# tdj28/ml-depth-pro-video

Measured on AMD Instinct MI355X. Metric: frames/sec at 1536x1536 (1/2/4/8 MI355X) + depth L1 vs reference, higher is better.
Workload: dtype bf16+f16; 1 GPU; BASELINE config 2/3: one 1536x1536 frame per GPU per step through DepthPro.infer (patch+image+FOV ViT-L, decoder, heads), hipGraph replay; global_batch=1, parallelism=frame-dp1, graph=True

## Files before the change

### ml-depth-pro-video_amd/csrc/dp_gemm.hip

```cpp
#include "dp_gemm_impl.h"

namespace dpg {
std::atomic<int> g_dbg_flags{0};

constexpr int DP_MAX_DEV = 64;
std::atomic<int> g_num_cu[DP_MAX_DEV];
int num_cus() {
  int dev = 0;
  if (hipGetDevice(&dev) != hipSuccess || dev < 0) dev = 0;
  std::atomic<int>& slot = g_num_cu[dev < DP_MAX_DEV ? dev : 0];
  int n = slot.load(std::memory_order_relaxed);
  if (n <= 0) {
    if (hipDeviceGetAttribute(&n, hipDeviceAttributeMultiprocessorCount, dev) != hipSuccess || n <= 0) n = 256;
    if (dev < DP_MAX_DEV) slot.store(n, std::memory_order_relaxed);
  }
  return n;
}
}

namespace {
int launch_tile(const GemmP& p, int tile, bool conv, bool bf16, hipStream_t s) {
  switch (tile) {
    case DP_TILE_PBIG_320x256: case DP_TILE_PBIG_256x256: return launch_part_pbig(p, tile, conv, bf16, s);
    case DP_TILE_256x64: case DP_TILE_256x32: case DP_TILE_128x128: case DP_TILE_DUAL_256x128:
// ... 19 lines not shown

namespace {
__global__ void ws_check_kernel(uint32_t* __restrict__ ws, int32_t* __restrict__ status) {
  const uint32_t err = ws[DP_GEMM_WS_ERROR_OFFSET / 4];
  if (threadIdx.x == 0) status[0] = (int32_t)err;
  if (err == 0) return;
  __syncthreads();
  for (int i = threadIdx.x; i < (int)(SK_FLAG_BYTES / 4); i += blockDim.x) ws[i] = 0u;
}
}

extern "C" int dp_gemm_workspace_check(void* workspace, int32_t* status, dp_stream_t stream) {
  if (!workspace || !status) return DP_ERR_ARG;
  hipLaunchKernelGGL(ws_check_kernel, dim3(1), dim3(256), 0, (hipStream_t)stream, (uint32_t*)workspace, status);
  DP_CHECK_LAUNCH();
  return 0;
}

namespace {
int gemm_plan(const dp_gemm_args* a, GemmP& p, int& tile) {
  if (!a) return DP_ERR_ARG;
  if (a->M <= 0 || a->N <= 0 || a->K <= 0) return DP_ERR_SHAPE;
  if (a->K % BK != 0 || a->N % 4 != 0) return DP_ERR_SHAPE;
  if (a->ldb % 8 != 0 || (a->a_mode == DP_A_DENSE && a->lda % 8 != 0)) return DP_ERR_ALIGN;
  if ((!a->head_w && a->store_mode != DP_STORE_HEAD_PS && a->ldc % 4 != 0) || (a->R1 && a->ldr1 % 4 != 0) ||
      (a->R2 && a->ldr2 % 4 != 0) || (a->pos && a->ldpos % 4 != 0))
    return DP_ERR_ALIGN;
  if (!a->A || !a->B || (!a->C && !a->ln_xl)) return DP_ERR_ARG;
  if (a->dtype != DP_BF16 && a->dtype != DP_F16) return DP_ERR_DTYPE;
  if (a->c_dtype != DP_BF16 && a->c_dtype != DP_F16 && a->c_dtype != DP_F32) return DP_ERR_DTYPE;
  if (a->c_dtype != DP_F32 && a->c_dtype != a->dtype) return DP_ERR_DTYPE;
  if (a->accumulate && a->c_dtype != DP_F32) return DP_ERR_DTYPE;
  if (a->pos && (a->pos_group <= 0)) return DP_ERR_ARG;
  if (a->a_mode == DP_A_CONV) {
    if (a->in_c % BK != 0 || a->k_h * a->k_w * a->in_c != a->K) return DP_ERR_SHAPE;
    if (a->out_h <= 0 || a->out_w <= 0 || a->stride <= 0 || a->M % (a->out_h * a->out_w) != 0)
      return DP_ERR_SHAPE;
  }
  if (a->store_mode == DP_STORE_HEAD_PS) {
    if (a->a_mode != DP_A_CONV || a->N != 128 || !a->head_w || !a->head_corr || a->c_dtype != DP_F32 ||
        a->accumulate || a->R1 || a->R2 || a->pos || a->gamma || a->act != DP_ACT_NONE)
      return DP_ERR_ARG;
  }
  if (a->store_mode == DP_STORE_ROWS && a->head_corr) {
    if (a->a_mode != DP_A_CONV || a->k_h != 3 || a->k_w != 3 || a->pad != 1 || a->stride != 1 || a->head_w ||
        a->relu_a ||
        a->row_group || a->out_h != a->in_h || a->out_w != a->in_w || a->N % 8 != 0 || a->N < 128 ||
        (a->tile != DP_TILE_AUTO && a->tile <= DP_TILE_256x32))
      return DP_ERR_ARG;
  }
  if (a->store_mode == DP_STORE_DECONV2X2) {
    if (a->dc_cout % 4 != 0 || a->N != 4 * a->dc_cout || a->dc_h <= 0 || a->dc_w <= 0 ||
        a->M % (a->dc_h * a->dc_w) != 0)
      return DP_ERR_SHAPE;
  }
  const bool lnp = a->ln_part_out || a->ln_xb_out || a->ln_xl || a->ln_rs_out,
             lnc = a->ln_part_in || a->ln_colsum || a->ln_rs_in;
  if (lnp && lnc) return DP_ERR_ARG;
  if (lnp && !a->ln_xl && (!a->ln_part_out || !a->ln_xb_out || !a->accumulate || !a->C || a->c_dtype != DP_F32 ||
                           a->act != DP_ACT_NONE || a->N % 256 != 0))
    return DP_ERR_ARG;
  if (a->ln_xl && (!a->ln_xb_out || !a->accumulate || a->c_dtype != DP_F32 || a->act != DP_ACT_NONE ||
                   a->N % 256 != 0 || a->ldc % 8 != 0 || (long long)a->M * a->ldc * 4 >= 0xFFFFFF00LL))
    return DP_ERR_ARG;
  if (lnc && (!(a->ln_part_in || a->ln_rs_in) || (a->ln_part_in && a->ln_rs_in) || !a->ln_colsum || a->K != 1024 ||
              a->accumulate || a->c_dtype == DP_F32 || a->gamma || (a->act != DP_ACT_NONE && a->act != DP_ACT_GELU) ||
              !(a->ln_eps > 0.f)))
    return DP_ERR_ARG;
  if (a->ln_rs_out && (!a->ln_xl || !a->ln_part_out || a->N != 1024 || !(a->ln_eps > 0.f) ||
                       !(a->workspace && a->workspace_bytes >= dp_gemm_workspace_size()) ||
                       (a->M + 319) / 320 > 1023 - LN_CNT_WORD))
    return DP_ERR_ARG;
  if (a->ln_rs_in && a->tile != DP_TILE_AUTO && a->tile != DP_TILE_P8PH_256x256) return DP_ERR_ARG;
  if ((lnp || lnc) && a->tile != DP_TILE_AUTO && a->tile != DP_TILE_8PH_320x256 &&
      !(lnc && a->tile == DP_TILE_P8PH_256x256))
    return DP_ERR_ARG;
  const bool ws_ok = a->workspace && a->workspace_bytes >= dp_gemm_workspace_size();
  const int dbg = g_dbg_flags.load(std::memory_order_relaxed);
  tile = a->tile;
  if (a->ln_rs_in) tile = DP_TILE_P8PH_256x256;
  if (a->store_mode == DP_STORE_HEAD_PS) {
    if (tile != DP_TILE_CV3_256x256 && tile != DP_TILE_CV3_384x128 && tile != DP_TILE_BIG_256x128)
      tile = a->M >= 512 * 256 ? DP_TILE_BIG_512x128 : DP_TILE_BIG_256x128;
  } else if (a->head_w) {
    if (a->N > 32 || a->store_mode != DP_STORE_ROWS) return DP_ERR_SHAPE;
    tile = DP_TILE_256x32;
  }
  const bool col8_shape = a->N % 8 == 0 && !(a->store_mode == DP_STORE_DECONV2X2 && a->dc_cout % 8 != 0);
  const bool col8_align = !(a->c_dtype != DP_F32 && a->ldc % 8 != 0) && !(a->R1 && a->ldr1 % 8 != 0) &&
                          !(a->R2 && a->ldr2 % 8 != 0);
  if (tile >= DP_TILE_BIG_256x256) {
    if (!col8_shape) return DP_ERR_SHAPE;
    if (!col8_align) return DP_ERR_ALIGN;
  }
  const long long tiles256 = (long long)((a->M + 255) / 256) * (a->N / 256);
  if (tile == DP_TILE_STREAMK_256x256 && (!ws_ok || a->N % 256 != 0)) return DP_ERR_ARG;
  if (tile == DP_TILE_AUTO) {
    if (a->N <= 32) tile = DP_TILE_256x32;
    else if (a->N <= 64) tile = DP_TILE_256x64;
    else if (!col8_shape || !col8_align) tile = DP_TILE_128x128;
    else if (a->N == 128 && a->M >= 512 * 256) {
      const bool cv3 = a->a_mode == DP_A_CONV && a->k_h == 3 && a->k_w == 3 && a->stride == 1 && a->pad == 1 &&
                       a->in_h == a->in_w && a->out_h == a->in_h && a->out_w == a->in_w && a->in_w % 16 == 0 &&
                       a->in_c % 64 == 0 && a->head_corr && a->store_mode == DP_STORE_ROWS && a->c_dtype != DP_F32 &&
                       !a->R1 && !a->R2 && !a->gamma && !a->pos && !a->accumulate && !a->row_group && !(dbg & 4096) &&
                       (long long)a->M * a->in_c < (1LL << 30);
      tile = !cv3 ? DP_TILE_BIG_512x128
             : a->in_w % 48 == 0 ? DP_TILE_CV3_384x128 : DP_TILE_CV3_256x256;
    }
    else if (a->N % 256 != 0) tile = DP_TILE_BIG_256x128;
    else if (ws_ok && a->a_mode == DP_A_CONV && !(dbg & 32) && tiles256 < num_cus() &&
             a->K >= 4608) {
      tile = DP_TILE_STREAMK_256x256;
    } else if (ws_ok && a->K <= 256 && tiles256 >= 1024) {
      tile = DP_TILE_STREAMK_256x256;
// ... 72 lines not shown
                        (a->accumulate && a->c_dtype == DP_F32 && a->act == DP_ACT_NONE);
    if (tile == DP_TILE_8PH_320x256 && !(plain && epi_ok)) return DP_ERR_ARG;
    if (plain && epi_ok) tile = DP_TILE_8PH_320x256;
  }
  if (a->tile == DP_TILE_AUTO && !(dbg & (1 << 16)) && a->a_mode == DP_A_CONV && a->k_h == 3 && a->k_w == 3 &&
      a->stride == 1 && a->pad == 1 && a->in_h == a->in_w && a->out_h == a->in_h && a->out_w == a->in_w &&
      a->in_w % 16 == 0 && a->in_c % 64 == 0 && a->N % 256 == 0 && a->store_mode == DP_STORE_ROWS &&
      !a->row_group && !a->head_w && !a->head_corr && (long long)a->M * a->in_c < (1LL << 30) && off32 &&
      a->c_dtype != DP_F32 && !a->gamma && !a->pos && !a->accumulate && a->act != DP_ACT_GELU && col8_align &&
      (long long)(a->M / 256) * (a->N / 256) >= 4LL * num_cus())
    tile = DP_TILE_CV3_256x256;
  else if (a->tile == DP_TILE_AUTO && !(dbg & (1 << 16)) && a->a_mode == DP_A_CONV &&
           a->k_h == 3 && a->k_w == 3 && a->stride == 1 && a->pad == 1 && a->in_h == a->in_w &&
           a->out_h == a->in_h && a->out_w == a->in_w && a->in_w % 16 == 0 && a->in_w % 12 == 0 &&
           a->in_c % 64 == 0 && a->N % 256 == 0 && a->store_mode == DP_STORE_ROWS && !a->row_group && !a->head_w &&
           !a->head_corr && (long long)a->M * a->in_c < (1LL << 30) && off32 && a->c_dtype != DP_F32 && !a->gamma &&
           !a->pos && !a->accumulate && a->act != DP_ACT_GELU && col8_align) {
    const long long t12 = (long long)(a->M / ((long long)a->in_w * a->in_w)) * (a->in_w / 12) * (a->in_w / 16) * (a->N / 256);
    const long long ncu = num_cus();
    if (t12 >= 2 * ncu && t12 % ncu == 0 && ((long long)(a->M / 256) * (a->N / 256)) % ncu != 0) tile = DP_TILE_CV3_192x256;
    else if (t12 <= ncu && 2 * t12 >= ncu) tile = DP_TILE_CV3_192x256;
  }
  if (tile >= DP_TILE_BIG_256x256 && !col8_shape) return DP_ERR_SHAPE;
  if (tile >= DP_TILE_BIG_256x256 && !col8_align) return DP_ERR_ALIGN;
  if (tile == DP_TILE_CV3_256x256 || tile == DP_TILE_CV3_192x256 || tile == DP_TILE_CV3_384x128) {
    const int th = tile == DP_TILE_CV3_192x256 ? 12 : tile == DP_TILE_CV3_384x128 ? 24 : 16, S = a->out_w;
    const bool hps = a->store_mode == DP_STORE_HEAD_PS, bc = a->store_mode == DP_STORE_ROWS && a->head_corr;
    if (a->a_mode != DP_A_CONV || a->k_h != 3 || a->k_w != 3 || a->stride != 1 || a->pad != 1 || a->in_h != S ||
        a->in_w != S || a->out_h != S || S % 16 != 0 || S % th != 0 || a->row_group || (a->head_w && !hps) || a->gamma ||
        a->pos || a->accumulate || (a->act != DP_ACT_NONE && a->act != DP_ACT_RELU) ||
        (long long)a->M * a->in_c >= (1LL << 30) || (long long)a->N * a->ldb >= (1LL << 31))
      return DP_ERR_ARG;
    if (!hps && a->store_mode != DP_STORE_ROWS) return DP_ERR_ARG;
    if (bc && (a->c_dtype == DP_F32 || a->R1 || a->R2 || a->N % 128 != 0)) return DP_ERR_ARG;
    if (!hps && !bc && (a->c_dtype == DP_F32 || a->N % 256 != 0)) return DP_ERR_ARG;
    if (th == 12 && (hps || bc)) return DP_ERR_ARG;
    if (th == 24 && !((hps || bc) && a->N == 128)) return DP_ERR_ARG;
  }
  if (a->store_mode == DP_STORE_ROWS && a->head_corr && tile != DP_TILE_BIG_512x128 && tile != DP_TILE_CV3_256x256 &&
      tile != DP_TILE_CV3_384x128)
    return DP_ERR_ARG;
  if (tile == DP_TILE_CV3_384x128 && (!a->head_corr || a->N != 128)) return DP_ERR_ARG;

  p.M = a->M; p.N = a->N; p.K = a->K;
  p.A = (const u16*)a->A; p.lda = a->lda;
  p.B = (const u16*)a->B; p.ldb = a->ldb;
  p.relu_a = a->relu_a;
  p.in_h = a->in_h; p.in_w = a->in_w; p.in_c = a->in_c; p.k_h = a->k_h; p.k_w = a->k_w;
  p.stride = a->stride; p.pad = a->pad; p.out_h = a->out_h; p.out_w = a->out_w;
  p.bias = a->bias; p.act = a->act; p.gamma = a->gamma;
  p.pos = a->pos; p.ldpos = a->ldpos; p.pos_group = a->pos_group; p.pos_off = a->pos_off;
  p.R1 = (const u16*)a->R1; p.ldr1 = a->ldr1; p.R2 = (const u16*)a->R2; p.ldr2 = a->ldr2;
  p.C = a->C; p.ldc = a->ldc; p.c_dtype = a->c_dtype; p.accumulate = a->accumulate;
  p.store_mode = a->store_mode; p.dc_h = a->dc_h; p.dc_w = a->dc_w; p.dc_cout = a->dc_cout;
  p.row_group = a->row_group; p.row_group_out = a->row_group_out; p.row_off = a->row_off;
  p.head_w = a->head_w; p.head_b = a->head_b; p.head_corr = a->head_corr;
  p.ln_part_out = a->ln_part_out; p.ln_xb_out = (u16*)a->ln_xb_out; p.ln_xl = (u16*)a->ln_xl;
  p.ln_part_in = a->ln_part_in; p.ln_colsum = a->ln_colsum; p.ln_eps = a->ln_eps;
  p.ln_rs = a->ln_rs_in;
  p.ln_rs_out = a->ln_rs_out;
  p.ln_cnt = a->ln_rs_out ? (unsigned*)a->workspace + LN_CNT_WORD : nullptr;
  p.tiles_n = 1;
  p.tiles_m = 1;
  if (tile == DP_TILE_STREAMK_256x256) {
    p.tiles_n = a->N / 256;
    p.tiles_m = (a->M + 255) / 256;
// ... 87 lines not shown
```

### ml-depth-pro-video_amd/csrc/dp_gemm_cv3.hip

```cpp
#include "dp_gemm_impl.h"

namespace {

constexpr int CV_TW = 16;
constexpr int CV_PW = CV_TW + 2;
template <int TH> struct CvGeo {
  static constexpr int PIX = (TH + 2) * CV_PW;
  static constexpr int PPW = (PIX * 8 + 511) / 512;
  static constexpr int PATCH_B = 8 * PPW * 1024;
  static constexpr int FM = TH / 2, HQ = FM / 2;
  static constexpr int NREAL = (PIX + 7) / 8;
  static constexpr bool TIGHT = NREAL * 1024 + ((FM + 1) * CV_PW + 2) * 128 < 65536;
  static constexpr int PSTRIDE = TIGHT ? NREAL * 1024 : PATCH_B;
  static constexpr int TRASH = 2 * PSTRIDE;
  static constexpr int WOFF = TIGHT ? 2 * PSTRIDE + 1024 : 2 * PATCH_B;
};

constexpr int CV_EPI_RES = 0, CV_EPI_BC = 1, CV_EPI_HPS = 2;
constexpr int CV_STAMPS = 16, CV_STAMP_WGS = 4096;
__device__ unsigned long long g_cv3_stamp[CV_STAMP_WGS * CV_STAMPS];
template <typename K_, bool RELU, int BN, int EPI, int ABL = 0, int TH = 16>
__global__ void __launch_bounds__(512, 1) gemm_cv3_kernel(const GemmP p) {
  using G = CvGeo<TH>;
  constexpr int FM = G::FM, HQ = G::HQ, PPW = G::PPW, CV_PATCH_B = G::PATCH_B, CV_PIX = G::PIX;
  constexpr bool TIGHT = G::TIGHT;
  constexpr int PSTRIDE = G::PSTRIDE, WOFF = G::WOFF;
  constexpr int TN = BN / 4, FN = TN / 16, QF = FN / 2;
  static_assert(TH == 16 || TH == 12 || (TH == 24 && BN == 128), "tile rows");
  constexpr int NBH = BN / 128;
  constexpr int B_B = BN * 128;
  static_assert(EPI != CV_EPI_RES || BN == 256, "residual epilogue: BN 256");
  static_assert(EPI != CV_EPI_HPS || BN == 128, "head epilogue: one parity (32 columns) per wave");
  __shared__ __attribute__((aligned(1024))) char smem[WOFF + 2 * B_B];

  const int tid = threadIdx.x, lane = tid & 63;
  const int wave = tid >> 6;
  const int wave_u = __builtin_amdgcn_readfirstlane(wave);
  unsigned long long st_[CV_STAMPS] = {};
  if constexpr ((ABL & 8) != 0) { st_[0] = __builtin_amdgcn_s_memtime(); st_[4] = __builtin_amdgcn_s_memrealtime(); }
  const int wm = wave >> 2, wn = wave & 3;
  const int nwg = gridDim.x, bid = blockIdx.x;
  const int xcd = bid & 7, q8 = nwg >> 3, r8 = nwg & 7;
  const int wgid = (xcd < r8 ? xcd * (q8 + 1) : r8 * (q8 + 1) + (xcd - r8) * q8) + (bid >> 3);
  const int S = p.out_w, tpr = S / CV_TW, tpi = (S / TH) * tpr;
  const int tn = wgid % p.tiles_n, sp = wgid / p.tiles_n;
  const int img = sp / tpi, r_ = sp - img * tpi;
  const int y0 = (r_ / tpr) * TH, x0 = (r_ % tpr) * CV_TW, n0 = tn * BN;
  const int cin = p.in_c, CB = cin / 64;
  const int KT = CB * 9;

  constexpr uint32_t CV_PAD = 0x80000000u;
  auto patch_off = [&](int i, int c0) __attribute__((always_inline)) {
    const int c = c0 + i * 64;
    const int P = c >> 3, slot = c & 7;
    uint32_t off = CV_PAD;
    if (P < CV_PIX) {
      const int pr = P / CV_PW, pc = P - pr * CV_PW;
      const int iy = y0 - 1 + pr, ix = x0 - 1 + pc;
      if ((unsigned)iy < (unsigned)S && (unsigned)ix < (unsigned)S)
        off = 2u * (uint32_t)(((img * S + iy) * S + ix) * cin + ((slot ^ (P & 7)) << 3));
    }
    return off;
  };
  const uint32_t lds0 = __builtin_amdgcn_readfirstlane(lds_addr(smem));
  const u32x4_t a_rs = raw_rsrc(p.A, (uint32_t)((long long)p.M * cin * 2));

  constexpr int HALF = 128 * 128;
  const int prow = wave * 8 + (lane >> 3);
  const int pchunk = (lane & 7) ^ ((lane >> 3) & 7);
  const uint32_t boff = 2u * (uint32_t)((n0 + prow) * (int)p.ldb + pchunk * 8);
  auto issue_b = [&](int h, int t) {
    const uint32_t dst = lds0 + WOFF + (t & 1) * B_B + h * HALF + wave_u * 1024;
    #pragma unroll
    for (int i = 0; i < 2; ++i) glds16s(boff, p.B + (long long)(h * 128 + i * 64) * p.ldb + 64 * t, dst + i * 8192);
  };
  auto issue_patch1 = [&](int cb, int buf, int i) {
    int c0 = wave * PPW * 64 + lane;
    asm volatile("" : "+v"(c0));
    const int j = wave_u * PPW + i;
    const uint32_t dst = lds0 + ((!TIGHT || j < G::NREAL) ? buf * PSTRIDE + j * 1024 : G::TRASH);
    glds16b(patch_off(i, c0) + cb * 128, a_rs, dst);
  };
  auto issue_patch3 = [&](int cb, int buf, int i0) {
    int c0 = wave * PPW * 64 + lane;
    asm volatile("" : "+v"(c0));
    #pragma unroll
    for (int i = i0; i < i0 + PPW / 2; ++i) {
      const int j = wave_u * PPW + i;
      const uint32_t dst = lds0 + ((!TIGHT || j < G::NREAL) ? buf * PSTRIDE + j * 1024 : G::TRASH);
      glds16b(patch_off(i, c0) + cb * 128, a_rs, dst);
    }
  };

  f32x4_t acc[FM][FN];
  #pragma unroll
  for (int i = 0; i < FM; ++i)
    #pragma unroll
    for (int j = 0; j < FN; ++j) acc[i][j] = f32x4_t{0.f, 0.f, 0.f, 0.f};
  const int frow = lane & 15, fchunk = lane >> 4;
  uint4 af[2][HQ], bf[2][2][QF];
  typedef __attribute__((address_space(3))) const char lds_c;
  typedef __attribute__((address_space(3))) const u32x4_t lds_u4;
  uint32_t abase[8][2], bbase[2];
  {
    const int PB = wm * FM * CV_PW + frow;
    #pragma unroll
    for (int v = 0; v < 8; ++v)
      #pragma unroll
      for (int ks = 0; ks < 2; ++ks) abase[v][ks] = lds0 + PB * 128 + (((ks * 4 + fchunk) ^ ((PB + v) & 7)) << 4);
    #pragma unroll
    for (int ks = 0; ks < 2; ++ks)
      bbase[ks] = lds0 + WOFF + (wn * TN + frow) * 128 + (((ks * 4 + fchunk) ^ (frow & 7)) << 4);
  }
  auto readA = [&](int qm, int ky, int kx, int pb) __attribute__((always_inline)) {
    const int boff_ = TIGHT ? pb * PSTRIDE : 0;
    #pragma unroll
    for (int ks = 0; ks < 2; ++ks)
      #pragma unroll
      for (int fm = 0; fm < HQ; ++fm) {
        const int c = (qm * HQ + fm + ky) * CV_PW + kx;
        af[ks][fm] = __builtin_bit_cast(uint4, *(lds_u4*)((lds_c*)(uintptr_t)abase[c & 7][ks] + boff_ + c * 128));
      }
    if constexpr (RELU && (ABL & 32)) {
      #pragma unroll
      for (int ks = 0; ks < 2; ++ks)
        #pragma unroll
        for (int fm = 0; fm < HQ; ++fm) af[ks][fm] = relu_pk16(af[ks][fm]);
      __builtin_amdgcn_sched_barrier(0);
    }
  };
  auto readB = [&](int qn, int st) __attribute__((always_inline)) {
    #pragma unroll
    for (int ks = 0; ks < 2; ++ks)
      #pragma unroll
      for (int fn = 0; fn < QF; ++fn)
        bf[qn][ks][fn] = __builtin_bit_cast(uint4, *(lds_u4*)((lds_c*)(uintptr_t)bbase[ks] + st * B_B + (qn * (TN / 2) + fn * 16) * 128));
  };
  int so_ = 0;
// ... 25 lines not shown
      __builtin_amdgcn_sched_barrier(0);
      #pragma unroll
      for (int ks = 0; ks < 2; ++ks)
        #pragma unroll
        for (int fm = 0; fm < HQ; ++fm) af[ks][fm] = relu_pk16(af[ks][fm]);
      __builtin_amdgcn_sched_barrier(0);
    }
  };
  auto bar = [&]() {
    const unsigned long long b0_ = tick();
    if constexpr ((ABL & 16) == 0) asm volatile("s_barrier" ::: "memory");
    if constexpr ((ABL & 256) != 0) st_[7 + so_] += tick() - b0_;
  };

  issue_patch3(0, 0, 0); issue_patch3(0, 0, PPW / 2);
  #pragma unroll
  for (int h = 0; h < NBH; ++h) issue_b(h, 0);
  if (KT > 1) {
    #pragma unroll
    for (int h = 0; h < NBH; ++h) issue_b(h, 1);
    wait_vmcnt<2 * NBH>();
  } else {
    wait_vmcnt<0>();
  }
  lds_barrier();
  if constexpr ((ABL & 8) != 0) st_[1] = __builtin_amdgcn_s_memtime();
  if constexpr ((ABL & 512) != 0) { if (wave_u >= 4) __builtin_amdgcn_s_setprio(1); }
  if (wm == 1) bar();
  int cb = 0;
  auto block = [&](auto st0_tag) __attribute__((always_inline)) {
    constexpr int ST0 = decltype(st0_tag)::value;
    constexpr int pb = ST0;
    const bool nb = cb + 1 < CB;
    #pragma unroll
    for (int tap = 0; tap < 9; ++tap) {
      const int ky = tap / 3, kx = tap - ky * 3, st = (ST0 + tap) & 1;
      const int t = cb * 9 + tap;
      const bool np = tap < PPW && nb;
      const bool n2 = t + 2 < KT;
      if constexpr ((ABL & 256) != 0) so_ = tap == 0 ? 4 : 0;
      const unsigned long long s0_ = tick();
      readA(0, ky, kx, pb); readB(0, st); readB(1, st);
      if (np && !(ABL & 2) && !(ABL & 128)) issue_patch1(cb + 1, pb ^ 1, tap);
      relu_early();
      bar(); mma(0, 0); mma(0, 1); bar();
      readA(1, ky, kx, pb);
      if (n2 && !(ABL & 2) && !(ABL & 64)) issue_b(0, t + 2);
      relu_early();
      const unsigned long long v0_ = tick();
      if (np) { if (n2) wait_vmcnt<1 + 2>(); else wait_vmcnt<1>(); }
      else { if (n2) wait_vmcnt<2>(); else wait_vmcnt<0>(); }
      if constexpr ((ABL & 256) != 0) st_[6 + so_] += tick() - v0_;
      if (NBH == 2 && n2 && !(ABL & 2) && !(ABL & 64)) issue_b(1, t + 2);
      bar(); mma(1, 0); mma(1, 1); bar();
      if constexpr ((ABL & 256) != 0) st_[tap == 0 ? 15 : 14] += tick() - s0_;
    }
    if constexpr (!TIGHT) {
      const uint32_t d = pb ? (uint32_t)-CV_PATCH_B : (uint32_t)CV_PATCH_B;
      #pragma unroll
      for (int v = 0; v < 8; ++v)
        #pragma unroll
        for (int ks = 0; ks < 2; ++ks) abase[v][ks] += d;
    }
    ++cb;
  };
  for (int pair = 0; pair < CB / 2; ++pair) {
    block(std::integral_constant<int, 0>{});
    block(std::integral_constant<int, 1>{});
  }
  if (CB & 1) block(std::integral_constant<int, 0>{});
  if (wm == 0) bar();
  if constexpr ((ABL & 512) != 0) __builtin_amdgcn_s_setprio(0);

  lds_barrier();
  if constexpr ((ABL & 8) != 0) st_[2] = __builtin_amdgcn_s_memtime();
  if constexpr ((ABL & 1) != 0) {
    float z = 0.f;
    #pragma unroll
    for (int i = 0; i < FM; ++i)
      #pragma unroll
      for (int j = 0; j < FN; ++j) z += acc[i][j][0];
    if (z == 1234.5f) ((float*)p.C)[tid] = z;
    return;
  }
  const int t = lane & 15, g = lane >> 4;
  const int nw = n0 + wn * TN;
  f32x4_t bias[FN];
  #pragma unroll
  for (int fn = 0; fn < FN; ++fn)
    bias[fn] = p.bias ? *(const f32x4_t*)(p.bias + nw + fn * 16 + 4 * g) : f32x4_t{0.f, 0.f, 0.f, 0.f};
  auto mrow = [&](int fm) { return (long long)((img * S + y0 + wm * FM + fm) * S + x0); };
  if constexpr (EPI == CV_EPI_HPS) {
    const int q = nw >> 5, dy = q >> 1, dx = q & 1;
    float hw[FN][4];
    #pragma unroll
    for (int fn = 0; fn < FN; ++fn)
      #pragma unroll
      for (int r = 0; r < 4; ++r) hw[fn][r] = p.head_w[(nw & 31) + fn * 16 + 4 * g + r];
    const long long W2 = 2LL * S;
    #pragma unroll 1
    for (int fm = 0; fm < FM; ++fm) {
      const int y = y0 + wm * FM + fm, x = x0 + t;
      float z[FN][4];
      #pragma unroll
      for (int fn = 0; fn < FN; ++fn)
        #pragma unroll
        for (int r = 0; r < 4; ++r) z[fn][r] = acc[fm][fn][r] + bias[fn][r];
      const bool top = y == 0 && dy == 0, bot = y == S - 1 && dy == 1;
      const bool lft = x == 0 && dx == 0, rgt = x == S - 1 && dx == 1;
      if (top || bot || lft || rgt) {
        #pragma unroll
        for (int a = 0; a < 3; ++a)
          #pragma unroll
          for (int c = 0; c < 3; ++c) {
            const bool oob = (a == 0 && top) || (a == 2 && bot) || (c == 0 && lft) || (c == 2 && rgt);
            if (oob) {
              #pragma unroll
              for (int fn = 0; fn < FN; ++fn)
                #pragma unroll
                for (int r = 0; r < 4; ++r) z[fn][r] -= p.head_corr[(a * 3 + c) * 32 + (nw & 31) + fn * 16 + 4 * g + r];
            }
          }
      }
      float hs = 0.f;
      #pragma unroll
      for (int fn = 0; fn < FN; ++fn)
        #pragma unroll
        for (int r = 0; r < 4; ++r) hs += fmaxf(z[fn][r], 0.f) * hw[fn][r];
      hs += __shfl_xor(hs, 16);
      hs += __shfl_xor(hs, 32);
      if (g == 0) ((float*)p.C)[((long long)img * 2 * S + 2 * y + dy) * W2 + 2 * x + dx] = fmaxf(hs + p.head_b, 0.f);
    }
  } else {
// ... 45 lines not shown
          if (p.R1) addr(xv, r1c[fn]);
          if (p.R2) addr(xv, r2c[fn]);
        }
        const int chunk = fn * 2 + (g >> 1);
        uint2 w;
        w.x = K_::pack2(xv[0], xv[1]);
        w.y = K_::pack2(xv[2], xv[3]);
        *(uint2*)(slab + t * (TN * 2) + ((chunk ^ (t & (CH - 1))) << 4) + (g & 1) * 8) = w;
      }
      #pragma unroll
      for (int k = 0; k < 16 / RPI; ++k) {
        const int row = k * RPI + lane / CH, chunk = lane % CH;
        const uint4 d = *(const uint4*)(slab + row * (TN * 2) + ((chunk ^ (row & (CH - 1))) << 4));
        *(uint4*)((u16*)p.C + (mrow(fm) + row) * p.ldc + nw + chunk * 8) = d;
      }
      if (fm + PD < FM) loadr(fm + PD, r1c, r2c);
    }
  }
  if constexpr ((ABL & 8) != 0) {
    asm volatile("s_waitcnt vmcnt(0)" ::: "memory");
    st_[3] = __builtin_amdgcn_s_memtime();
    st_[5] = __builtin_amdgcn_s_memrealtime();
    if (tid == 0 && blockIdx.x < CV_STAMP_WGS) {
      #pragma unroll
      for (int k = 0; k < CV_STAMPS; ++k) g_cv3_stamp[blockIdx.x * CV_STAMPS + k] = st_[k];
    }
  }
}

template <typename K_>
int launch_cv3(const GemmP& p0, hipStream_t s, int th) {
  GemmP p = p0;
  const int S = p.out_w;
  if (p.k_h != 3 || p.k_w != 3 || p.stride != 1 || p.pad != 1 || p.in_h != S || p.in_w != S || p.out_h != S ||
      S % CV_TW || S % th || p.in_c % 64 || p.M % (S * S) || p.row_group || (p.head_w && p.store_mode != DP_STORE_HEAD_PS) ||
      p.gamma || p.pos || p.accumulate || (p.act != DP_ACT_NONE && p.act != DP_ACT_RELU))
    return DP_ERR_ARG;
  if ((long long)p.M * p.in_c >= (1LL << 30) || (long long)p.N * p.ldb >= (1LL << 31)) return DP_ERR_ARG;
  int epi, bn;
  if (p.store_mode == DP_STORE_HEAD_PS) {
    if (p.N != 128 || !p.head_w || !p.head_corr || p.c_dtype != DP_F32 || p.R1 || p.R2 || p.act) return DP_ERR_ARG;
    epi = CV_EPI_HPS; bn = 128;
  } else if (p.store_mode == DP_STORE_ROWS && p.head_corr) {
    if (p.c_dtype == DP_F32 || p.R1 || p.R2 || p.N % 128) return DP_ERR_ARG;
    epi = CV_EPI_BC; bn = p.N % 256 ? 128 : 256;
  } else if (p.store_mode == DP_STORE_ROWS) {
    if (p.c_dtype == DP_F32 || p.N % 256) return DP_ERR_ARG;
    epi = CV_EPI_RES; bn = 256;
  } else {
    return DP_ERR_ARG;
  }
  if (th == 12 && epi != CV_EPI_RES) return DP_ERR_ARG;
  if (th == 24 && ((epi != CV_EPI_BC && epi != CV_EPI_HPS) || bn != 128)) return DP_ERR_ARG;
  p.tiles_n = p.N / bn;
  p.tiles_m = (p.M / (S * S)) * (S / th) * (S / CV_TW);
  dim3 grid(p.tiles_m * p.tiles_n);
  const int abl = (p.dbg & (1 << 24)) ? p.dbg & 2047 : 0;
  if (th == 24) {
    if (epi == CV_EPI_BC && !p.relu_a && abl == 8) hipLaunchKernelGGL((gemm_cv3_kernel<K_, false, 128, CV_EPI_BC, 8, 24>), grid, dim3(512), 0, s, p);
    else if (epi == CV_EPI_BC && !p.relu_a && abl == 264) hipLaunchKernelGGL((gemm_cv3_kernel<K_, false, 128, CV_EPI_BC, 264, 24>), grid, dim3(512), 0, s, p);
    else if (epi == CV_EPI_HPS) hipLaunchKernelGGL((gemm_cv3_kernel<K_, false, 128, CV_EPI_HPS, 0, 24>), grid, dim3(512), 0, s, p);
    else if (p.relu_a) hipLaunchKernelGGL((gemm_cv3_kernel<K_, true, 128, CV_EPI_BC, 0, 24>), grid, dim3(512), 0, s, p);
    else hipLaunchKernelGGL((gemm_cv3_kernel<K_, false, 128, CV_EPI_BC, 0, 24>), grid, dim3(512), 0, s, p);
    DP_CHECK_LAUNCH();
    return 0;
  }
  if (th == 12) {
    if (abl == 8 && p.relu_a) hipLaunchKernelGGL((gemm_cv3_kernel<K_, true, 256, CV_EPI_RES, 8, 12>), grid, dim3(512), 0, s, p);
    else if (abl == 1032 && p.relu_a) hipLaunchKernelGGL((gemm_cv3_kernel<K_, true, 256, CV_EPI_RES, 1032, 12>), grid, dim3(512), 0, s, p);
    else if (abl == 520 && p.relu_a) hipLaunchKernelGGL((gemm_cv3_kernel<K_, true, 256, CV_EPI_RES, 520, 12>), grid, dim3(512), 0, s, p);
    else if (abl == 264 && p.relu_a) hipLaunchKernelGGL((gemm_cv3_kernel<K_, true, 256, CV_EPI_RES, 264, 12>), grid, dim3(512), 0, s, p);
    else if (p.relu_a) hipLaunchKernelGGL((gemm_cv3_kernel<K_, true, 256, CV_EPI_RES, 0, 12>), grid, dim3(512), 0, s, p);
    else hipLaunchKernelGGL((gemm_cv3_kernel<K_, false, 256, CV_EPI_RES, 0, 12>), grid, dim3(512), 0, s, p);
    DP_CHECK_LAUNCH();
    return 0;
  }
#define DP_CV3(B_, E_) do { \
    if (p.relu_a) hipLaunchKernelGGL((gemm_cv3_kernel<K_, true, B_, E_>), grid, dim3(512), 0, s, p); \
    else hipLaunchKernelGGL((gemm_cv3_kernel<K_, false, B_, E_>), grid, dim3(512), 0, s, p); } while (0)
  if (epi == CV_EPI_RES && abl && p.relu_a) {
    switch (abl) {
#define DP_CV3A(A_) case A_: hipLaunchKernelGGL((gemm_cv3_kernel<K_, true, 256, CV_EPI_RES, A_>), grid, dim3(512), 0, s, p); break;
      DP_CV3A(1) DP_CV3A(2) DP_CV3A(3) DP_CV3A(4) DP_CV3A(5) DP_CV3A(6) DP_CV3A(7) DP_CV3A(8)
      DP_CV3A(10) DP_CV3A(12) DP_CV3A(14) DP_CV3A(24) DP_CV3A(26) DP_CV3A(28) DP_CV3A(30) DP_CV3A(40) DP_CV3A(72)
      DP_CV3A(136) DP_CV3A(264) DP_CV3A(520) DP_CV3A(1032)
#undef DP_CV3A
      default: DP_CV3(256, CV_EPI_RES);
    }
  } else if (epi == CV_EPI_RES) DP_CV3(256, CV_EPI_RES);
  else if (epi == CV_EPI_HPS) DP_CV3(128, CV_EPI_HPS);
// ... 21 lines not shown
```

### ml-depth-pro-video_amd/depth_pro/engine.py

```python

from __future__ import annotations

import os
from typing import Dict, Optional, Tuple

import torch

from . import ops
from ._lib import (DP_ACT_GELU, DP_ACT_RELU, DP_BF16, DP_F16, DP_F32, DP_TILE_P8PH_256x256, DP_TILE_SPLITK_256x256,
                   DPError, load)
from .spec import DEPTH, EMBED_DIM, HEADS, IMG_SIZE, MLP_DIM, TOKENS

_ABLATE = set(filter(None, os.environ.get("DP_ABLATE", "").split(",")))


def ln_fold_enabled() -> bool:
    return not ({"ln", "vitgemm"} & _ABLATE)


NWIN = 35
TOK = TOKENS
PTOK = TOKENS - 1
D = EMBED_DIM


def _conv_w(w: torch.Tensor, dt) -> torch.Tensor:
    return ops.conv_weight(w, dt)


def _deconv_w(w: torch.Tensor, dt) -> torch.Tensor:
    ci, co = w.shape[0], w.shape[1]
    return w.permute(2, 3, 1, 0).reshape(4 * co, ci).to(dt).contiguous()


def _f32(t: torch.Tensor) -> torch.Tensor:
    return t.detach().to(torch.float32).contiguous()


def compose_head(wd: torch.Tensor, bd: torch.Tensor, w2: torch.Tensor, b2: torch.Tensor, dt) -> Dict[str, object]:
    ci_n, c_n = wd.shape[0], wd.shape[1]
    o_n = w2.shape[0]
    wc = torch.zeros(4, o_n, 3, 3, ci_n, dtype=torch.float32, device=wd.device)
    for dy in range(2):
        for dx in range(2):
            q = 2 * dy + dx
            for a in range(-1, 2):
                ry = dy + a
                ty, py = ry // 2 + 1, ry & 1
                for b in range(-1, 2):
                    rx = dx + b
                    tx, px = rx // 2 + 1, rx & 1
                    wc[q, :, ty, tx, :] += w2[:, :, a + 1, b + 1] @ wd[:, :, py, px].t()
    corr = torch.einsum("ocab,c->abo", w2, bd).contiguous()
    bias = (b2 + corr.sum(dim=(0, 1))).repeat(4).contiguous()
    w_conv = wc.reshape(4 * o_n, 3, 3, ci_n).permute(0, 3, 1, 2)
    return {"head.ps.w": ops.conv_weight(w_conv, dt), "head.ps.b": bias,
            "head.ps.corr": corr.reshape(-1).contiguous()}


def compose_head0(w0: torch.Tensor, b0: torch.Tensor, wo: torch.Tensor, bo: torch.Tensor, dt) -> Dict[str, object]:
    wc = torch.einsum("omyx,mc->ocyx", w0, wo)
    corr = torch.einsum("omyx,m->yxo", w0, bo).contiguous()
    bias = (b0 + corr.sum(dim=(0, 1))).contiguous()
    return {"head.0c.w": ops.conv_weight(wc, dt), "head.0c.b": bias, "head.0c.corr": corr.reshape(-1).contiguous()}


def precision_codes(codes) -> Tuple[int, int]:
    if isinstance(codes, (tuple, list)):
        v, d = int(codes[0]), int(codes[1])
    else:
        v = d = int(codes)
    for c in (v, d):
        if c not in (DP_BF16, DP_F16):
            raise DPError("compute dtype must be bf16 or f16")
    return v, d


def pack_weights(sd: Dict[str, torch.Tensor], device: torch.device, dtype_code) -> Dict[str, object]:
    vcode, dcode = precision_codes(dtype_code)
    vdt, dt = ops.torch_dtype(vcode), ops.torch_dtype(dcode)
    g = lambda k: sd[k].detach().to(device)
    P: Dict[str, object] = {}
    fold = ln_fold_enabled()
    for vit in ("encoder.patch_encoder.", "encoder.image_encoder.", "fov.encoder.0."):
        if vit + "cls_token" not in sd:
            continue
        folded = fold and vit == "encoder.patch_encoder."
        P[vit + "cls"] = _f32(g(vit + "cls_token")).reshape(D)
        P[vit + "pos"] = _f32(g(vit + "pos_embed")).reshape(TOK, D)
        P[vit + "pe.w"] = g(vit + "patch_embed.proj.weight").reshape(D, -1).to(vdt).contiguous()
# ... 201 lines not shown
        self.t384_256 = e(384 * 384, 256)
        self.enc0 = e(768 * 768, 256)
        self.t96_256b = e(96 * 96, 256)
        self.t192_256b = e(192 * 192, 256)
        self.enc1 = e(384 * 384, 256)
        self.t96_512 = e(96 * 96, 512)
        self.enc2 = e(192 * 192, 512)
        self.t48_1024 = e(48 * 48, D)
        self.enc3 = e(96 * 96, D)
        self.t24_1024 = e(24 * 24, D)
        self.cat = e(48 * 48, 2 * D)
        self.enc4 = e(48 * 48, D)
        self.dec = {}
        for s in (48, 96, 192, 384, 768):
            self.dec[s] = {k: e(s * s, 256) for k in ("c", "t", "x", "y")}
        self.low = self.dec[48]["c"]
        self.up = {s: e(s * s, 256) for s in (96, 192, 384, 768)}
        self.feats = e(768 * 768, 256)
        self.h0 = e(768 * 768, 128)
        self.canonical = e(1, 1, S, S, dtype=torch.float32)
        self.fov_tok = e(PTOK, 128)
        self.fx = e(24 * 24, 128)
        self.f12 = e(12 * 12, 64)
        self.f6 = e(6 * 6, 32)
        self.fov_deg = e(1, 1, 1, 1, dtype=torch.float32)
        self.graph: Optional[torch.cuda.CUDAGraph] = None
        self.side = torch.cuda.Stream(device=dev)
        self.dec_a = torch.cuda.Stream(device=dev)
        self.dec_b = torch.cuda.Stream(device=dev)
        self.dec_c = torch.cuda.Stream(device=dev)
        self.ws_main = ops.gemm_workspace(dev)
        self.ws_dec = ops.gemm_workspace(dev)
        self.head0_compose = os.environ.get("DP_HEAD0_COMPOSE", "1") == "1" and "head.0c.w" in packed
        self.qkv_gamma = ops.log2q_gamma(HEADS, D // HEADS, dev)
        self.serial_side = False
        self._wss = [self.ws_main, self.ws_dec]
        self.status_dev = torch.zeros(len(self._wss) + 1, dtype=torch.int32, device=dev)
        self._frames = 0
        self._recent: list = []
        self._unreported: list = []
        self.last_status: Optional[FrameStatus] = None
        self.sync_check = os.environ.get("DP_CHECK_SYNC", "0") == "1"
        self.qkv_tile = DP_TILE_P8PH_256x256

    def _vit(self, pres, buf: _ViTBuffers, n_img: int, cols_off_rows: int, hooks=None):
        for _ in self._vit_steps(pres, buf, n_img, cols_off_rows, hooks):
            pass

    def _vit_steps(self, pres, buf: _ViTBuffers, n_img: int, cols_off_rows: int, hooks=None):
        P, M = self.P, n_img * TOK
        G = len(pres)
        ln_on = "ln" not in _ABLATE and not (G > 1 and "sideln" in _ABLATE)
        gemm_on = "vitgemm" not in _ABLATE

        def lin(A, key, C, N, K, a_rows=True, **kw):
            per = {k: kw.pop(k) for k in ("bias", "gamma", "pos") if isinstance(kw.get(k), str)}
            A_off = kw.pop("A_off", 0)
            groups = []
            for g, pre in enumerate(pres):
                d = dict(A=A, B=P[pre + key], C=C, A_off=A_off + (g * M * K if a_rows else 0), C_off=g * M * N)
                d.update({k: P[pre + v] for k, v in per.items()})
                groups.append(d)
            ops.gemm_grouped(groups, M=kw.pop("M", M), N=N, K=K, **kw)

        def norm(key, out):
            ops.layernorm_grouped(buf.x, [P[pre + key + ".weight"] for pre in pres],
# ... 210 lines not shown
                self.dec_c.wait_event(ev["lat0pre"])
            self._deconv(self.t384_256, 384, 256, P[e + "upsample_latent0.3"], self.enc0, 256)
            ev["enc0"] = mark(self.dec_c)
            if early:
                self._resblock_head("decoder.fusions.0.resnet1", self.enc0, 768, t1)
                ev["r1a"] = mark(self.dec_c)
            if self.use_fov and side_ok:
                if not serial:
                    self.dec_c.wait_stream(self.side)
                self._fov_head()
        if "decoder" not in _ABLATE:
            f = self._fusion(4, self.low, 48, None)
            for i, s in ((3, 96), (2, 192), (1, 384)):
                if not serial:
                    main.wait_event(ev[f"c{i}"])
                    if i == 1:
                        main.wait_event(ev["enc0"])
                f = self._fusion(i, f, s, self.dec[s]["c"])
            if early and not serial:
                main.wait_event(ev["r1a"])
            feats = self._fusion(0, f, 768, self.enc0, t1=t1)
        else:
            feats = self.feats
        if not serial:
            for st in (self.dec_a, self.dec_b, self.dec_c, self.side):
                main.wait_stream(st)
        if "head" in _ABLATE:
            return self.canonical, self.fov_deg
        if self.head0_compose and "decoder" not in _ABLATE:
            self._conv3(feats, 768, 256, P["head.0c.w"], self.h0, 128, bias=P["head.0c.b"],
                        border_corr=P["head.0c.corr"])
        else:
            self._conv3(feats, 768, 256, P["head.0.w"], self.h0, 128, bias=P["head.0.b"])
        ops.gemm(self.h0, P["head.ps.w"], self.canonical, M=768 * 768, N=128, K=9 * 128,
                 conv=dict(in_h=768, in_w=768, in_c=128, k=3, stride=1, pad=1, out_h=768, out_w=768),
                 bias=P["head.ps.b"], head_w=P["head.4.w"], head_b=P["head.4.b"], head_corr=P["head.ps.corr"])
        return self.canonical, self.fov_deg

    def capture_graph(self) -> None:
        s = torch.cuda.Stream(device=self.dev)
        s.wait_stream(torch.cuda.current_stream(self.dev))
        with torch.cuda.stream(s):
            self.forward()
        torch.cuda.current_stream(self.dev).wait_stream(s)
        g = torch.cuda.CUDAGraph()
        with torch.cuda.graph(g):
            self.forward()
        self.graph = g

    def run(self) -> Tuple[torch.Tensor, torch.Tensor]:
        if self.graph is not None:
            self.graph.replay()
        else:
            self.forward()
        return self.canonical, self.fov_deg

    def finish_status(self) -> FrameStatus:
        words = torch.empty(self.status_dev.numel(), dtype=torch.int32, pin_memory=True)
        words.copy_(self.status_dev, non_blocking=True)
        self.status_dev[-1:].zero_()
        ev = torch.cuda.Event()
        ev.record()
        st = FrameStatus(self._frames, words, ev)
        self._frames += 1
        self._recent.append(st)
        if len(self._recent) > 64:
            self._sweep(block_oldest=True)
# ... 41 lines not shown
```

Measured before the change: 52.78 frames/sec.

## Compact head pixel-shuffle conv to four taps per parity instead of nine

```diff
diff --git a/ml-depth-pro-video_amd/csrc/dp_gemm.hip b/ml-depth-pro-video_amd/csrc/dp_gemm.hip
--- a/ml-depth-pro-video_amd/csrc/dp_gemm.hip
+++ b/ml-depth-pro-video_amd/csrc/dp_gemm.hip
@@ -75,8 +75,10 @@
   if (a->c_dtype != DP_F32 && a->c_dtype != a->dtype) return DP_ERR_DTYPE;
   if (a->accumulate && a->c_dtype != DP_F32) return DP_ERR_DTYPE;
   if (a->pos && (a->pos_group <= 0)) return DP_ERR_ARG;
+  const bool hps4 = a->a_mode == DP_A_CONV && a->store_mode == DP_STORE_HEAD_PS && a->k_h == 3 && a->k_w == 3 &&
+                    a->stride == 1 && a->pad == 1 && a->K == 4 * a->in_c;
   if (a->a_mode == DP_A_CONV) {
-    if (a->in_c % BK != 0 || a->k_h * a->k_w * a->in_c != a->K) return DP_ERR_SHAPE;
+    if (a->in_c % BK != 0 || (a->k_h * a->k_w * a->in_c != a->K && !hps4)) return DP_ERR_SHAPE;
     if (a->out_h <= 0 || a->out_w <= 0 || a->stride <= 0 || a->M % (a->out_h * a->out_w) != 0)
       return DP_ERR_SHAPE;
   }
@@ -123,7 +125,10 @@
   tile = a->tile;
   if (a->ln_rs_in) tile = DP_TILE_P8PH_256x256;
   if (a->store_mode == DP_STORE_HEAD_PS) {
-    if (tile != DP_TILE_CV3_256x256 && tile != DP_TILE_CV3_384x128 && tile != DP_TILE_BIG_256x128)
+    if (hps4) {
+      if (tile == DP_TILE_AUTO) tile = a->out_w % 48 == 0 ? DP_TILE_CV3_384x128 : DP_TILE_CV3_256x256;
+      else if (tile != DP_TILE_CV3_256x256 && tile != DP_TILE_CV3_384x128) return DP_ERR_ARG;
+    } else if (tile != DP_TILE_CV3_256x256 && tile != DP_TILE_CV3_384x128 && tile != DP_TILE_BIG_256x128)
       tile = a->M >= 512 * 256 ? DP_TILE_BIG_512x128 : DP_TILE_BIG_256x128;
   } else if (a->head_w) {
     if (a->N > 32 || a->store_mode != DP_STORE_ROWS) return DP_ERR_SHAPE;
@@ -262,6 +267,7 @@
         (long long)a->M * a->in_c >= (1LL << 30) || (long long)a->N * a->ldb >= (1LL << 31))
       return DP_ERR_ARG;
     if (!hps && a->store_mode != DP_STORE_ROWS) return DP_ERR_ARG;
+    if (hps4 && a->relu_a) return DP_ERR_ARG;
     if (bc && (a->c_dtype == DP_F32 || a->R1 || a->R2 || a->N % 128 != 0)) return DP_ERR_ARG;
     if (!hps && !bc && (a->c_dtype == DP_F32 || a->N % 256 != 0)) return DP_ERR_ARG;
     if (th == 12 && (hps || bc)) return DP_ERR_ARG;
diff --git a/ml-depth-pro-video_amd/csrc/dp_gemm_cv3.hip b/ml-depth-pro-video_amd/csrc/dp_gemm_cv3.hip
--- a/ml-depth-pro-video_amd/csrc/dp_gemm_cv3.hip
+++ b/ml-depth-pro-video_amd/csrc/dp_gemm_cv3.hip
@@ -19,8 +19,10 @@
 constexpr int CV_EPI_RES = 0, CV_EPI_BC = 1, CV_EPI_HPS = 2;
 constexpr int CV_STAMPS = 16, CV_STAMP_WGS = 4096;
 __device__ unsigned long long g_cv3_stamp[CV_STAMP_WGS * CV_STAMPS];
-template <typename K_, bool RELU, int BN, int EPI, int ABL = 0, int TH = 16>
+template <typename K_, bool RELU, int BN, int EPI, int ABL = 0, int TH = 16, int NT = 9>
 __global__ void __launch_bounds__(512, 1) gemm_cv3_kernel(const GemmP p) {
+  constexpr bool CPT = NT == 4;
+  static_assert(NT == 9 || (CPT && EPI == CV_EPI_HPS), "taps per channel block");
   using G = CvGeo<TH>;
   constexpr int FM = G::FM, HQ = G::HQ, PPW = G::PPW, CV_PATCH_B = G::PATCH_B, CV_PIX = G::PIX;
   constexpr bool TIGHT = G::TIGHT;
@@ -47,7 +49,7 @@
   const int img = sp / tpi, r_ = sp - img * tpi;
   const int y0 = (r_ / tpr) * TH, x0 = (r_ % tpr) * CV_TW, n0 = tn * BN;
   const int cin = p.in_c, CB = cin / 64;
-  const int KT = CB * 9;
+  const int KT = CB * NT;
 
   constexpr uint32_t CV_PAD = 0x80000000u;
   auto patch_off = [&](int i, int c0) __attribute__((always_inline)) {
@@ -69,10 +71,11 @@
   const int prow = wave * 8 + (lane >> 3);
   const int pchunk = (lane & 7) ^ ((lane >> 3) & 7);
   const uint32_t boff = 2u * (uint32_t)((n0 + prow) * (int)p.ldb + pchunk * 8);
+  auto kcol = [&](int t) { return CPT ? (t & 3) * cin + (t >> 2) * 64 : 64 * t; };
   auto issue_b = [&](int h, int t) {
     const uint32_t dst = lds0 + WOFF + (t & 1) * B_B + h * HALF + wave_u * 1024;
     #pragma unroll
-    for (int i = 0; i < 2; ++i) glds16s(boff, p.B + (long long)(h * 128 + i * 64) * p.ldb + 64 * t, dst + i * 8192);
+    for (int i = 0; i < 2; ++i) glds16s(boff, p.B + (long long)(h * 128 + i * 64) * p.ldb + kcol(t), dst + i * 8192);
   };
   auto issue_patch1 = [&](int cb, int buf, int i) {
     int c0 = wave * PPW * 64 + lane;
@@ -103,7 +106,7 @@
   typedef __attribute__((address_space(3))) const u32x4_t lds_u4;
   uint32_t abase[8][2], bbase[2];
   {
-    const int PB = wm * FM * CV_PW + frow;
+    const int PB = wm * FM * CV_PW + frow + (CPT ? (wn >> 1) * CV_PW + (wn & 1) : 0);
     #pragma unroll
     for (int v = 0; v < 8; ++v)
       #pragma unroll
@@ -195,23 +198,31 @@
     constexpr int ST0 = decltype(st0_tag)::value;
     constexpr int pb = ST0;
     const bool nb = cb + 1 < CB;
-    #pragma unroll
-    for (int tap = 0; tap < 9; ++tap) {
-      const int ky = tap / 3, kx = tap - ky * 3, st = (ST0 + tap) & 1;
-      const int t = cb * 9 + tap;
-      const bool np = tap < PPW && nb;
+    constexpr int NS = PPW < NT - 1 ? PPW : NT - 1;
+    #pragma unroll
+    for (int tap = 0; tap < NT; ++tap) {
+      const int ky = CPT ? tap >> 1 : tap / 3, kx = CPT ? tap & 1 : tap - ky * 3;
+      const int st = CPT ? tap & 1 : (ST0 + tap) & 1;
+      const int t = cb * NT + tap;
+      const bool np = tap < NS && nb;
+      const int pi0 = tap * PPW / NS, pn = (tap + 1) * PPW / NS - pi0;
       const bool n2 = t + 2 < KT;
       if constexpr ((ABL & 256) != 0) so_ = tap == 0 ? 4 : 0;
       const unsigned long long s0_ = tick();
       readA(0, ky, kx, pb); readB(0, st); readB(1, st);
-      if (np && !(ABL & 2) && !(ABL & 128)) issue_patch1(cb + 1, pb ^ 1, tap);
+      if (np && !(ABL & 2) && !(ABL & 128)) {
+        #pragma unroll
+        for (int i = 0; i < pn; ++i) issue_patch1(cb + 1, pb ^ 1, pi0 + i);
+      }
       relu_early();
       bar(); mma(0, 0); mma(0, 1); bar();
       readA(1, ky, kx, pb);
       if (n2 && !(ABL & 2) && !(ABL & 64)) issue_b(0, t + 2);
       relu_early();
       const unsigned long long v0_ = tick();
-      if (np) { if (n2) wait_vmcnt<1 + 2>(); else wait_vmcnt<1>(); }
+      if (np && pn == 3) { if (n2) wait_vmcnt<3 + 2>(); else wait_vmcnt<3>(); }
+      else if (np && pn == 2) { if (n2) wait_vmcnt<2 + 2>(); else wait_vmcnt<2>(); }
+      else if (np) { if (n2) wait_vmcnt<1 + 2>(); else wait_vmcnt<1>(); }
       else { if (n2) wait_vmcnt<2>(); else wait_vmcnt<0>(); }
       if constexpr ((ABL & 256) != 0) st_[6 + so_] += tick() - v0_;
       if (NBH == 2 && n2 && !(ABL & 2) && !(ABL & 64)) issue_b(1, t + 2);
@@ -261,7 +272,7 @@
       #pragma unroll
       for (int r = 0; r < 4; ++r) hw[fn][r] = p.head_w[(nw & 31) + fn * 16 + 4 * g + r];
     const long long W2 = 2LL * S;
-    #pragma unroll 1
+    #pragma unroll
     for (int fm = 0; fm < FM; ++fm) {
       const int y = y0 + wm * FM + fm, x = x0 + t;
       float z[FN][4];
@@ -373,6 +384,9 @@
 int launch_cv3(const GemmP& p0, hipStream_t s, int th) {
   GemmP p = p0;
   const int S = p.out_w;
+  const bool cpt = p.store_mode == DP_STORE_HEAD_PS && p.K == 4 * p.in_c;
+  if (!cpt && p.K != 9 * p.in_c) return DP_ERR_ARG;
+  if (cpt && (p.relu_a || th == 12)) return DP_ERR_ARG;
   if (p.k_h != 3 || p.k_w != 3 || p.stride != 1 || p.pad != 1 || p.in_h != S || p.in_w != S || p.out_h != S ||
       S % CV_TW || S % th || p.in_c % 64 || p.M % (S * S) || p.row_group || (p.head_w && p.store_mode != DP_STORE_HEAD_PS) ||
       p.gamma || p.pos || p.accumulate || (p.act != DP_ACT_NONE && p.act != DP_ACT_RELU))
@@ -397,6 +411,12 @@
   p.tiles_m = (p.M / (S * S)) * (S / th) * (S / CV_TW);
   dim3 grid(p.tiles_m * p.tiles_n);
   const int abl = (p.dbg & (1 << 24)) ? p.dbg & 2047 : 0;
+  if (cpt) {
+    if (th == 24) hipLaunchKernelGGL((gemm_cv3_kernel<K_, false, 128, CV_EPI_HPS, 0, 24, 4>), grid, dim3(512), 0, s, p);
+    else hipLaunchKernelGGL((gemm_cv3_kernel<K_, false, 128, CV_EPI_HPS, 0, 16, 4>), grid, dim3(512), 0, s, p);
+    DP_CHECK_LAUNCH();
+    return 0;
+  }
   if (th == 24) {
     if (epi == CV_EPI_BC && !p.relu_a && abl == 8) hipLaunchKernelGGL((gemm_cv3_kernel<K_, false, 128, CV_EPI_BC, 8, 24>), grid, dim3(512), 0, s, p);
     else if (epi == CV_EPI_BC && !p.relu_a && abl == 264) hipLaunchKernelGGL((gemm_cv3_kernel<K_, false, 128, CV_EPI_BC, 264, 24>), grid, dim3(512), 0, s, p);
diff --git a/ml-depth-pro-video_amd/depth_pro/engine.py b/ml-depth-pro-video_amd/depth_pro/engine.py
--- a/ml-depth-pro-video_amd/depth_pro/engine.py
+++ b/ml-depth-pro-video_amd/depth_pro/engine.py
@@ -54,8 +54,21 @@
     corr = torch.einsum("ocab,c->abo", w2, bd).contiguous()
     bias = (b2 + corr.sum(dim=(0, 1))).repeat(4).contiguous()
     w_conv = wc.reshape(4 * o_n, 3, 3, ci_n).permute(0, 3, 1, 2)
-    return {"head.ps.w": ops.conv_weight(w_conv, dt), "head.ps.b": bias,
+    return {"head.ps.w": ops.conv_weight(w_conv, dt), "head.ps.w4": compact_head_w(wc, dt), "head.ps.b": bias,
             "head.ps.corr": corr.reshape(-1).contiguous()}
+
+
+def compact_head_w(wc: torch.Tensor, dt) -> torch.Tensor:
+    q_n, o_n, _, _, ci_n = wc.shape
+    out = torch.empty(q_n, o_n, 4, ci_n, dtype=torch.float32, device=wc.device)
+    for q in range(q_n):
+        dy, dx = q >> 1, q & 1
+        keep = torch.zeros(3, 3, dtype=torch.bool, device=wc.device)
+        keep[dy:dy + 2, dx:dx + 2] = True
+        if wc[q][:, ~keep].ne(0).any():
+            raise AssertionError(f"composed head conv: parity {q} has a non-zero weight outside its 2 x 2 taps")
+        out[q] = wc[q][:, dy:dy + 2, dx:dx + 2].reshape(o_n, 4, ci_n)
+    return out.reshape(q_n * o_n, 4 * ci_n).to(dt).contiguous()
 
 
 def compose_head0(w0: torch.Tensor, b0: torch.Tensor, wo: torch.Tensor, bo: torch.Tensor, dt) -> Dict[str, object]:
@@ -323,6 +336,7 @@
         self.ws_main = ops.gemm_workspace(dev)
         self.ws_dec = ops.gemm_workspace(dev)
         self.head0_compose = os.environ.get("DP_HEAD0_COMPOSE", "1") == "1" and "head.0c.w" in packed
+        self.head_ps_compact = os.environ.get("DP_HEAD_PS_COMPACT", "1") == "1" and "head.ps.w4" in packed
         self.qkv_gamma = ops.log2q_gamma(HEADS, D // HEADS, dev)
         self.serial_side = False
         self._wss = [self.ws_main, self.ws_dec]
@@ -599,7 +613,9 @@
                         border_corr=P["head.0c.corr"])
         else:
             self._conv3(feats, 768, 256, P["head.0.w"], self.h0, 128, bias=P["head.0.b"])
-        ops.gemm(self.h0, P["head.ps.w"], self.canonical, M=768 * 768, N=128, K=9 * 128,
+        taps = 4 if self.head_ps_compact else 9
+        ops.gemm(self.h0, P["head.ps.w4" if self.head_ps_compact else "head.ps.w"], self.canonical,
+                 M=768 * 768, N=128, K=taps * 128,
                  conv=dict(in_h=768, in_w=768, in_c=128, k=3, stride=1, pad=1, out_h=768, out_w=768),
                  bias=P["head.ps.b"], head_w=P["head.4.w"], head_b=P["head.4.b"], head_corr=P["head.ps.corr"])
         return self.canonical, self.fov_deg
```

New measurement: 53.32 frames/sec, median of 6. 1.01x the previous value.
